# bababyVN/medical-image-segmentation-and-classification

Measured on AMD Instinct MI355X. Metric: images/sec (train step) Attention U-Net 256x256 bs=32/GPU, higher is better.
Workload: dtype bf16; 1 GPU; AttentionUNet 256x256 train step (fwd+BCE+bwd+clip+AdamW), bs=32/GPU, NHWC bf16 activations, fp32 master weights; global_batch=32, parallelism=dp1, hip_graph=False, wgrad_side_stream=True, plan_replay=C (mi355_plan_run)

## Files before the change

### include/mi355conv.h

```cpp
#ifndef MI355CONV_H_
#define MI355CONV_H_

#include <stdint.h>

#ifdef __cplusplus
extern "C" {
#endif

typedef struct ihipStream_t* mi355_stream_t;

enum { MI355_F32 = 0, MI355_BF16 = 1, MI355_F16 = 2 };
enum { MI355_OK = 0, MI355_ERR_ARG = -1, MI355_ERR_UNSUPPORTED = -2, MI355_ERR_RUNTIME = -3 };

int mi355_version(void);
const char* mi355_last_error(void);


int mi355_pack_input_nchw(const float* x, void* y, int N, int C, int H, int W, int Cpad, int dtype,
                          mi355_stream_t s);
int mi355_pack_input_im2col3(const float* x, void* y, int N, int C, int H, int W, int dtype, mi355_stream_t s);
int mi355_unpack_output_nchw(const void* x, float* y, int N, int C, int H, int W, int ld, int dtype,
                             mi355_stream_t s);
int mi355_pack_nchw(const float* x, void* y, int N, int C, int H, int W, int ld, int dtype, mi355_stream_t s);

int mi355_pack_conv_weight(const float* w, void* wf, void* wb, int Co, int Ci, int Cip, int KH, int KW,
                           int transposed, int dtype, mi355_stream_t s);

int mi355_pack_conv_weights_batched(const int64_t* table, int n, int fields ,
                                    int dtype, mi355_stream_t s);

int mi355_conv2d_igemm(const void* in, const void* wk, const float* bias, void* out,
                       int N, int Hi, int Wi, int Ci, int ldi,
                       int Ho, int Wo, int Co, int ldo,
                       int KH, int KW, int mul, int kmul, int off, int div, int up,
                       int accumulate, float* stats, int dtype, mi355_stream_t s);
int mi355_conv2d_igemm_variant(int Hi, int Wi, int Ci, int Ho, int Wo, int Co, int KH, int KW, int mul, int kmul, int off,
                               int div, int up, int dtype);
int mi355_conv2d_igemm_variant_n(int N, int Hi, int Wi, int Ci, int Ho, int Wo, int Co, int KH, int KW, int mul, int kmul,
                                 int off, int div, int up, int dtype);
int mi355_conv2d_igemm_dma_tile(int N, int Ho, int Wo, int Ci, int Co);
int mi355_conv2d_igemm_generic_tile(int N, int Ho, int Wo, int Co);
int mi355_conv2d_igemm_stat_rows(int N, int Hi, int Wi, int Ci, int Ho, int Wo, int Co, int KH, int KW,
                                 int mul, int kmul, int off, int div, int up, int dtype);
int mi355_conv2d_igemm_pool2_ok(int N, int Hi, int Wi, int Ci, int Ho, int Wo, int Co, int KH, int KW,
                                int mul, int kmul, int off, int div, int up, int dtype);
const char* mi355_conv2d_igemm_kernel_name(int N, int Hi, int Wi, int Ci, int Ho, int Wo, int Co, int KH, int KW,
                                           int mul, int kmul, int off, int div, int up, int dtype);

int mi355_conv2d_wgrad_splits(int N, int Ho, int Wo, int Ci, int Co, int KH, int KW);
int mi355_conv2d_wgrad_variant(int N, int Ho, int Wo, int KH, int KW, int stride, int pad, int dtype);
const char* mi355_conv2d_wgrad_kernel_name(int N, int Ho, int Wo, int Ci, int Co, int KH, int KW, int stride, int pad, int dtype);
int mi355_conv2d_wgrad(const void* x, const void* dy, float* ws, int splits,
                       int N, int Hi, int Wi, int Ci, int ldx,
                       int Ho, int Wo, int Co, int ldy,
                       int KH, int KW, int stride, int pad, int up, int dtype, mi355_stream_t s);
int mi355_conv2d_wgrad_multi_ok(int N, int Ho, int Wo, int dtype);
int mi355_conv2d_wgrad_multi(const void* x0, const void* dy0, const void* x1, const void* dy1, const void* x2, const void* dy2,
                             const void* x3, const void* dy3, const void* x4, const void* dy4, const void* x5, const void* dy5,
                             int napp, float* ws, int splits, int N, int Hi, int Wi, int Ci, int ldx, int Ho, int Wo, int Co,
                             int ldy, int up, int dtype, mi355_stream_t s);
int mi355_conv2d_wgrad_reduce(const float* ws, int splits, float* dw, int Co, int Ci, int Ci_real,
                              int KH, int KW, int transposed, float beta, mi355_stream_t s);


int mi355_rowreduce_blocks(long long M);
int mi355_bn_stats(const void* x, float* partial, long long M, int C, int ld, int dtype, mi355_stream_t s);
int mi355_bn_finalize(const float* partial, int nblocks, long long M, int C, const float* gamma,
                      const float* beta, float* running_mean, float* running_var, int64_t* nbt,
                      float momentum, float eps, float* scale, float* shift, float* mean, float* invstd,
                      mi355_stream_t s);
int mi355_fold_rows(const float* partial, int rows, int rowlen, float* out, int nsplit, mi355_stream_t s);
int mi355_bn_fold_bias(const float* bias, const float* scale, const float* shift, float* out, int C, mi355_stream_t s);
int mi355_bn_eval_coeffs(const float* gamma, const float* beta, const float* running_mean,
                         const float* running_var, float eps, int C, float* scale, float* shift,
                         mi355_stream_t s);
int mi355_bn_act(const void* x, int ldx, const float* scale, const float* shift,
                 const void* x2, int ldx2, const float* scale2, const float* shift2,
                 const void* res, int ldr, void* y, int ldy, long long M, int C, int act, int dtype,
                 mi355_stream_t s);
int mi355_bn_act_pool2(const void* x, int ldx, const float* scale, const float* shift, void* y, int ldy, void* p, int ldp,
                       int N, int H, int W, int C, int act, int dtype, mi355_stream_t s);
int mi355_bn_act_windows(const void* x, int ldx, const float* scale, const float* shift, const void* res, int ldr, void* y, int ldy,
                         int N, int H, int W, int C, int act, int dtype, mi355_stream_t s);
int mi355_bn_bwd_reduce_rows(long long M);
int mi355_bn_bwd_reduce(const void* dy, int lddy, const void* y, int ldy, const void* x, int ldx,
                        const float* mean, const float* invstd, const float* mscale, const float* mshift,
                        float* partial, long long M, int C, int act, int dtype, mi355_stream_t s);
int mi355_bn_bwd_finalize(const float* partial, int nblocks, int C, float* sums, float* dgamma, float* dbeta,
                          float acc, mi355_stream_t s);
int mi355_bn_bwd_finalize_at(const float* partial, int nblocks, int nq, int q0, int q1, int C, float* sums, float* dgamma,
                             float* dbeta, float acc, mi355_stream_t s);
int mi355_bn_bwd_apply(const void* dy, int lddy, const void* y, int ldy, const void* x, int ldx,
                       const float* gamma, const float* mean, const float* invstd, const float* mscale,
                       const float* mshift, const float* sums, void* dx, int lddx, void* dres, int lddres,
                       void* dpost, int lddpost, int post_acc, float* dbias_partial,
                       long long M, int C, int act, int dtype, mi355_stream_t s);
int mi355_bn_bwd_apply_post4(const void* dy, int lddy, const void* y, int ldy, const void* x, int ldx,
                             const float* gamma, const float* mean, const float* invstd, const float* mscale,
                             const float* mshift, const float* sums, void* dx, int lddx, void* dpost, int lddpost,
                             int post_acc, const void* ex0, const void* ex1, const void* ex2, const void* ex3, int ldex,
                             long long M, int C, int act, int dtype, mi355_stream_t s);
int mi355_bn_bwd_pool2_ok(int H, int W, int C, int dtype);
int mi355_bn_bwd_reduce_pool2_rows(long long M);
int mi355_bn_bwd_reduce_pool2(const void* dy, int lddy, const void* dp, int lddp, const void* x, int ldx, const float* mean,
                              const float* invstd, const float* mscale, const float* mshift, float* partial,
                              int N, int H, int W, int C, int dtype, mi355_stream_t s);
int mi355_bn_bwd_apply_pool2(const void* dy, int lddy, const void* dp, int lddp, const void* x, int ldx, const float* gamma,
                             const float* mean, const float* invstd, const float* mscale, const float* mshift,
                             const float* sums, void* dx, int lddx, int N, int H, int W, int C, int dtype, mi355_stream_t s);
int mi355_colsum_finalize(const float* partial, int nblocks, int stride, int C, float* out, float acc,
                          mi355_stream_t s);
int mi355_colsum(const void* x, int ld, float* partial, long long M, int C, int dtype, mi355_stream_t s);

int mi355_maxpool_fwd(const void* x, int ldx, void* y, int ldy, int N, int H, int W, int C,
                      int k, int stride, int pad, int dtype, mi355_stream_t s);
int mi355_maxpool_bwd(const void* x, int ldx, const void* dy, int lddy, void* dx, int lddx,
                      int N, int H, int W, int C, int k, int stride, int pad, int accumulate, int dtype,
                      mi355_stream_t s);
int mi355_upsample2_bwd(const void* dy, int lddy, void* dx, int lddx, int N, int H, int W, int C,
                        int accumulate, int dtype, mi355_stream_t s);
int mi355_add(const void* a, int lda, const void* b, int ldb, void* y, int ldy, long long M, int C, int dtype,
              mi355_stream_t s);
int mi355_relu_fwd(const void* x, int ldx, void* y, int ldy, long long M, int C, int dtype, mi355_stream_t s);
int mi355_relu_bwd(const void* dy, int lddy, const void* y, int ldy, void* dx, int lddx, long long M, int C,
                   int dtype, mi355_stream_t s);

int mi355_rowdot_fwd(const void* x, int ldx, const float* w, const float* b, float* z, float* partial,
                     long long M, int C, int HW, int K, int dtype, mi355_stream_t s);
int mi355_rowdot_bwd(const float* dz, const void* x, int ldx, const float* w, void* dx, int lddx,
                     float* partial, long long M, int C, int relu_mask, int HW, int K, int accumulate, int dtype,
                     mi355_stream_t s);
int mi355_gate_mul_fwd(const void* x, int ldx, const float* z, const float* scale, const float* shift,
                       void* y, int ldy, long long M, int C, int dtype, mi355_stream_t s);
int mi355_gate_mul_bwd(const void* dy, int lddy, const void* x, int ldx, const float* z, const float* scale,
// ... 125 lines not shown
```

### medical-image-segmentation-and-classification_amd/csrc/conv_wgrad.hip

```cpp
#include "common.hpp"
#include "dma.hpp"
#include "wgrad3x3_halo.hpp"
#include "wgrad3x3_halo8.hpp"
#include <stdlib.h>

struct WgradArgs {
  const void* x;
  const void* dy;
  float* ws;
  int N, Hi, Wi, Ci, ldx;
  int Ho, Wo, Co, ldy;
  int KH, KW, stride, pad, up;
  int M, Hlog, Wlog;
  int chunk;
};

typedef __attribute__((address_space(3))) s16x4 lds_s16x4;
template <typename T> struct TwoByte { typedef T type; };
template <> struct TwoByte<float> { typedef bf16_t type; };

template <typename T, int BCO, int BCI>
__global__ __launch_bounds__(256) void conv_wgrad_kernel(const WgradArgs a) {
  constexpr int BP = 32;
  constexpr int EPC = 16 / (int)sizeof(T);
  constexpr bool BF = sizeof(T) == 2;
  constexpr int PO = BF ? (BCO == 128 ? 320 : 192) : BCO * 4;
  constexpr int PX = BF ? (BCI == 128 ? 320 : 192) : BCI * 4;
  constexpr int O_BYTES = BP * PO, X_BYTES = BP * PX, STAGE = O_BYTES + X_BYTES;
  constexpr int CPRO = BCO / EPC, CPRX = BCI / EPC;
  constexpr int O_IT = BP * CPRO / 256, X_IT = BP * CPRX / 256;
  constexpr int WTO = BCO / 2, WTI = BCI / 2;
  constexpr int MI = WTO / 32, NI = WTI / 32;
  static_assert(O_IT >= 1 && X_IT >= 1, "tile too small for 256 threads");
  __shared__ __attribute__((aligned(16))) unsigned char lds[2 * STAGE];

  const int tid = threadIdx.x, lane = tid & 63, wave = tid >> 6;
  const int r32 = lane & 31, h = lane >> 5;
  const int wo_ = wave >> 1, wi_ = wave & 1;
  const int ciTiles = (a.Ci + BCI - 1) / BCI;
  int bid = xcd_tile((blockIdx.z * gridDim.y + blockIdx.y) * gridDim.x + blockIdx.x, gridDim.x * gridDim.y * gridDim.z);
  const int bx = bid % gridDim.x; bid /= gridDim.x;
  const int co0 = (bx / ciTiles) * BCO, ci0 = (bx % ciTiles) * BCI;
  const int tap = bid % gridDim.y, kh = tap / a.KW, kw = tap - kh * a.KW;
  const int split = bid / gridDim.y;
  const int p_begin = split * a.chunk;
  const int p_end = min(a.M, p_begin + a.chunk);
  const T* __restrict__ x = reinterpret_cast<const T*>(a.x);
  const T* __restrict__ dy = reinterpret_cast<const T*>(a.dy);

  int o_row[O_IT], o_c[O_IT];
#pragma unroll
  for (int i = 0; i < O_IT; ++i) {
    const int id = tid + i * 256;
    o_row[i] = id / CPRO;
    o_c[i] = id - o_row[i] * CPRO;
  }
  int x_row[X_IT], x_c[X_IT], x_n[X_IT], x_ho[X_IT], x_wo[X_IT];
  const int HoWo = a.Ho * a.Wo;
#pragma unroll
  for (int i = 0; i < X_IT; ++i) {
    const int id = tid + i * 256;
    x_row[i] = id / CPRX;
    x_c[i] = id - x_row[i] * CPRX;
    const int m = p_begin + x_row[i];
    x_n[i] = m / HoWo;
    const int rem = m - x_n[i] * HoWo;
    x_ho[i] = rem / a.Wo;
    x_wo[i] = rem - x_ho[i] * a.Wo;
  }

  uint4 ro[O_IT], rx[X_IT];
  auto load_tile = [&](int p0) {
#pragma unroll
    for (int i = 0; i < O_IT; ++i) {
      const int m = p0 + o_row[i];
      const int c = co0 + o_c[i] * EPC;
      if (m < p_end && c < a.Co)
        ro[i] = *reinterpret_cast<const uint4*>(dy + (size_t)m * a.ldy + c);
      else
        ro[i] = make_uint4(0, 0, 0, 0);
    }
#pragma unroll
    for (int i = 0; i < X_IT; ++i) {
      const int m = p0 + x_row[i];
      const int c = ci0 + x_c[i] * EPC;
      int th = x_ho[i] * a.stride + kh - a.pad, tw = x_wo[i] * a.stride + kw - a.pad;
// ... 152 lines not shown
  const long long max_by_pixels = M / 256 > 0 ? M / 256 : 1;
  if (s > max_by_pixels) s = max_by_pixels;
  const long long slab = (long long)Co * KH * KW * Ci * 4;
  while (s > 1 && s * slab > (512ll << 20)) --s;
  if (s < 1) s = 1;
  return (int)s;
}

template <typename T>
static int wgrad_launch(const WgradArgs& a, int splits, hipStream_t s) {
  int bco, bci;
  wgrad_tiles(a.Co, a.Ci, bco, bci);
  dim3 grid(ceil_div(a.Co, bco) * ceil_div(a.Ci, bci), a.KH * a.KW, splits);
  if (bco == 128 && bci == 128)
    hipLaunchKernelGGL((conv_wgrad_kernel<T, 128, 128>), grid, dim3(256), 0, s, a);
  else if (bco == 128)
    hipLaunchKernelGGL((conv_wgrad_kernel<T, 128, 64>), grid, dim3(256), 0, s, a);
  else if (bci == 128)
    hipLaunchKernelGGL((conv_wgrad_kernel<T, 64, 128>), grid, dim3(256), 0, s, a);
  else
    hipLaunchKernelGGL((conv_wgrad_kernel<T, 64, 64>), grid, dim3(256), 0, s, a);
  MI355_LAUNCH_CHECK();
  return MI355_OK;
}

template <typename T, bool W16>
static int launch_wgrad3x3(const Wgrad3Args& h, dim3 grid, hipStream_t s) {
  constexpr int lds_bytes = Wgrad3Lds<W16>::BYTES;
  static const hipError_t configured =
      hipFuncSetAttribute((const void*)wgrad3x3_halo_kernel<T, W16>, hipFuncAttributeMaxDynamicSharedMemorySize, lds_bytes);
  if (configured != hipSuccess)
    MI355_FAIL((int)configured, "wgrad3x3_halo: cannot reserve %d B of LDS: %s", lds_bytes, hipGetErrorString(configured));
  hipLaunchKernelGGL((wgrad3x3_halo_kernel<T, W16>), grid, dim3(256), lds_bytes, s, h);
  MI355_LAUNCH_CHECK();
  return MI355_OK;
}
template <typename T, bool W32>
static int launch_wgrad3x3_8(const Wgrad3Args& h, dim3 grid, hipStream_t s) {
  constexpr int lds_bytes = Wgrad8Lds::BYTES;
  static const hipError_t configured =
      hipFuncSetAttribute((const void*)wgrad3x3_halo8_kernel<T, W32>, hipFuncAttributeMaxDynamicSharedMemorySize, lds_bytes);
  if (configured != hipSuccess)
    MI355_FAIL((int)configured, "wgrad3x3_halo8: cannot reserve %d B of LDS: %s", lds_bytes, hipGetErrorString(configured));
  hipLaunchKernelGGL((wgrad3x3_halo8_kernel<T, W32>), grid, dim3(512), lds_bytes, s, h);
  MI355_LAUNCH_CHECK();
  return MI355_OK;
}
static int wgrad3_mode(int N, int Ho, int Wo, int KH, int KW, int stride, int pad, int dtype) {
  static const int use_halo = getenv("MI355_WGRAD_HALO") ? atoi(getenv("MI355_WGRAD_HALO")) : 1;
  if (!use_halo || !dtype_is_2byte(dtype) || stride != 1 || pad != 1) return 0;
  return halo_wgrad_mode(N, Ho, Wo, KH, KW);
}
static bool wgrad3_launchable(int hmode, int Hi, int Wi, int ldx, int Ho, int Wo, int ldy, int up, int esz) {
  const long long img_lim = (1ll << 31) / (hmode == 2 || hmode == 4 ? 2 : 1);
  return Ho == (up ? 2 * Hi : Hi) && Wo == (up ? 2 * Wi : Wi) && (long long)Hi * Wi * ldx * esz < img_lim && (long long)Ho * Wo * ldy * esz < img_lim;
}

static Wgrad3Args fill_wgrad3(const void* const* xs, const void* const* dys, int napp, float* ws, int hmode, int splits, int N, int Hi,
                              int Wi, int Ci, int ldx, int Ho, int Wo, int Co, int ldy, int up) {
  Wgrad3Args h;
  for (int i = 0; i < 6; ++i) { h.xs[i] = xs[i < napp ? i : 0]; h.dys[i] = dys[i < napp ? i : 0]; }
  h.ws = ws;
  h.N = N; h.Hi = Hi; h.Wi = Wi; h.Ci = Ci; h.ldx = ldx;
  h.H = Ho; h.W = Wo; h.Co = Co; h.ldy = ldy; h.up = up ? 1 : 0;
  h.RB = Ho % 32 == 0 ? 32 : (Ho % 16 == 0 ? 16 : 8);
  h.items_per_app = halo_wgrad_items(hmode, N, Ho, Wo, h.RB);
  h.items = napp * h.items_per_app;
  h.items_per_block = ceil_div(h.items, splits);
  return h;
}

static const char* wgrad3_name(int hmode) { return hmode >= 3 ? "wgrad3x3_halo8_kernel" : "wgrad3x3_halo_kernel"; }
static int launch_wgrad3(const Wgrad3Args& h, int splits, int hmode, int dtype, hipStream_t s) {
  const dim3 grid(ceil_div(h.Co, 64) * ceil_div(h.Ci, 64), splits);
  const bool f16 = dtype == MI355_F16;
  switch (hmode) {
    case 2: return f16 ? launch_wgrad3x3<f16_t, true>(h, grid, s) : launch_wgrad3x3<bf16_t, true>(h, grid, s);
    case 3: return f16 ? launch_wgrad3x3_8<f16_t, false>(h, grid, s) : launch_wgrad3x3_8<bf16_t, false>(h, grid, s);
    case 4: return f16 ? launch_wgrad3x3_8<f16_t, true>(h, grid, s) : launch_wgrad3x3_8<bf16_t, true>(h, grid, s);
    default: return f16 ? launch_wgrad3x3<f16_t, false>(h, grid, s) : launch_wgrad3x3<bf16_t, false>(h, grid, s);
  }
}

extern "C" int mi355_conv2d_wgrad_variant(int N, int Ho, int Wo, int KH, int KW, int stride, int pad, int dtype) {
  return wgrad3_mode(N, Ho, Wo, KH, KW, stride, pad, dtype);
}
extern "C" int mi355_conv2d_wgrad_multi_ok(int N, int Ho, int Wo, int dtype) { return wgrad3_mode(N, Ho, Wo, 3, 3, 1, 1, dtype) ? 1 : 0; }
extern "C" const char* mi355_conv2d_wgrad_kernel_name(int N, int Ho, int Wo, int Ci, int Co, int KH, int KW, int stride, int pad, int dtype) {
  static thread_local char name[48];
  if (const int hmode = wgrad3_mode(N, Ho, Wo, KH, KW, stride, pad, dtype)) return wgrad3_name(hmode);
  int bco, bci;
  wgrad_tiles(Co, Ci, bco, bci);
  snprintf(name, sizeof(name), "conv_wgrad_kernel<%s,%d,%d>", dtype_is_2byte(dtype) ? "bf16" : "f32", bco, bci);
  return name;
}

extern "C" int mi355_conv2d_wgrad(const void* x, const void* dy, float* ws, int splits, int N, int Hi, int Wi, int Ci,
                                  int ldx, int Ho, int Wo, int Co, int ldy, int KH, int KW, int stride, int pad, int up,
                                  int dtype, mi355_stream_t s) {
  MI355_CHECK_ARG(x && dy && ws, "conv2d_wgrad: null pointer");
  MI355_CHECK_ARG(splits >= 1 && splits <= 65535, "conv2d_wgrad: splits=%d out of range", splits);
  const int esz = dtype_is_2byte(dtype) ? 2 : 4;
  const int epc = 16 / esz;
  MI355_CHECK_ARG(Ci % epc == 0 && Co % epc == 0, "conv2d_wgrad: Ci=%d / Co=%d must be multiples of %d", Ci, Co, epc);
  MI355_CHECK_ARG(((uintptr_t)x % 16) == 0 && ((uintptr_t)dy % 16) == 0 && (ldx * esz) % 16 == 0 && (ldy * esz) % 16 == 0,
                  "conv2d_wgrad: pointers / channel strides must be 16-byte aligned");
  MI355_CHECK_ARG((long long)N * Ho * Wo < (1ll << 31) && (long long)N * Hi * Wi < (1ll << 31),
                  "conv2d_wgrad: pixel count overflows int32");
  const int hmode = wgrad3_mode(N, Ho, Wo, KH, KW, stride, pad, dtype);
  if (hmode && wgrad3_launchable(hmode, Hi, Wi, ldx, Ho, Wo, ldy, up, esz))
    return launch_wgrad3(fill_wgrad3(&x, &dy, 1, ws, hmode, splits, N, Hi, Wi, Ci, ldx, Ho, Wo, Co, ldy, up), splits, hmode, dtype, (hipStream_t)s);
  WgradArgs a;
  a.x = x; a.dy = dy; a.ws = ws;
  a.N = N; a.Hi = Hi; a.Wi = Wi; a.Ci = Ci; a.ldx = ldx;
  a.Ho = Ho; a.Wo = Wo; a.Co = Co; a.ldy = ldy;
  a.KH = KH; a.KW = KW; a.stride = stride; a.pad = pad; a.up = up ? 1 : 0;
  a.M = N * Ho * Wo; a.Hlog = up ? 2 * Hi : Hi; a.Wlog = up ? 2 * Wi : Wi;
  a.chunk = ceil_div(ceil_div(a.M, splits), 32) * 32;
  return dispatch_dtype(dtype, "conv2d_wgrad", [&](auto tag) { return wgrad_launch<decltype(tag)>(a, splits, (hipStream_t)s); });
}

extern "C" int mi355_conv2d_wgrad_multi(const void* x0, const void* dy0, const void* x1, const void* dy1, const void* x2,
                                        const void* dy2, const void* x3, const void* dy3, const void* x4, const void* dy4,
                                        const void* x5, const void* dy5, int napp, float* ws, int splits, int N, int Hi, int Wi,
                                        int Ci, int ldx, int Ho, int Wo, int Co, int ldy, int up, int dtype, mi355_stream_t s) {
  const void* xs[6] = {x0, x1, x2, x3, x4, x5};
  const void* dys[6] = {dy0, dy1, dy2, dy3, dy4, dy5};
  MI355_CHECK_ARG(napp >= 1 && napp <= 6 && ws && splits >= 1, "conv2d_wgrad_multi: 1..6 operand pairs, a workspace, splits >= 1");
  for (int i = 0; i < napp; ++i)
    MI355_CHECK_ARG(xs[i] && dys[i] && ((uintptr_t)xs[i] % 16) == 0 && ((uintptr_t)dys[i] % 16) == 0,
                    "conv2d_wgrad_multi: pair %d: null or misaligned pointer", i);
  const int hmode = wgrad3_mode(N, Ho, Wo, 3, 3, 1, 1, dtype);
  MI355_CHECK_ARG(hmode, "conv2d_wgrad_multi: shape / dtype not served by the nine-tap kernel "
                  "(mi355_conv2d_wgrad_multi_ok == 0): run mi355_conv2d_wgrad per pair");
  MI355_CHECK_ARG(Ci % 8 == 0 && Co % 8 == 0 && (ldx * 2) % 16 == 0 && (ldy * 2) % 16 == 0 && ldx >= Ci && ldy >= Co,
                  "conv2d_wgrad_multi: channel counts / strides must be multiples of 8 elements");
  MI355_CHECK_ARG((up ? (Ho == 2 * Hi && Wo == 2 * Wi) : (Ho == Hi && Wo == Wi)), "conv2d_wgrad_multi: 3x3 / stride 1 / pad 1 geometry only");
  MI355_CHECK_ARG((long long)Hi * Wi * ldx * 4 < (1ll << 31) && (long long)Ho * Wo * ldy * 4 < (1ll << 31),
                  "conv2d_wgrad_multi: an image of 1 GiB or more is beyond the 32-bit offsets of the nine-tap kernel's buffer descriptors");
  const Wgrad3Args h = fill_wgrad3(xs, dys, napp, ws, hmode, splits, N, Hi, Wi, Ci, ldx, Ho, Wo, Co, ldy, up);
  MI355_CHECK_ARG(splits <= h.items, "conv2d_wgrad_multi: more splits (%d) than work items (%d)", splits, h.items);
  return launch_wgrad3(h, splits, hmode, dtype, (hipStream_t)s);
}


#define WR_CI 32
template <int TAPS>
__global__ __launch_bounds__(1024) void wgrad_reduce_kernel(const float* __restrict__ ws, int splits, float* __restrict__ dw, int Co,
                                                            int Ci, int Ci_real, int taps_rt, int transposed, float beta, int KL) {
  extern __shared__ float tile[];
  const int taps = TAPS > 0 ? TAPS : taps_rt;
  const int ciTiles = (Ci + WR_CI - 1) / WR_CI;
  const int co = blockIdx.x / ciTiles, ci0 = (blockIdx.x % ciTiles) * WR_CI;
  const size_t total = (size_t)Co * taps * Ci;
  const int cl = threadIdx.x % WR_CI, kl = threadIdx.x / WR_CI;
  const int ci = ci0 + cl;
  const int tstride = taps * (WR_CI + 1);
  if constexpr (TAPS > 0) {
    float s0[TAPS], s1[TAPS];
#pragma unroll
    for (int tap = 0; tap < TAPS; ++tap) { s0[tap] = 0.f; s1[tap] = 0.f; }
    if (ci < Ci) {
      const float* p = ws + (size_t)co * TAPS * Ci + ci;
      int k = kl;
      for (; k + KL < splits; k += 2 * KL) {
        float a[TAPS], b[TAPS];
#pragma unroll
        for (int tap = 0; tap < TAPS; ++tap) {
          a[tap] = p[(size_t)k * total + (size_t)tap * Ci];
          b[tap] = p[(size_t)(k + KL) * total + (size_t)tap * Ci];
        }
#pragma unroll
        for (int tap = 0; tap < TAPS; ++tap) { s0[tap] += a[tap]; s1[tap] += b[tap]; }
      }
      if (k < splits) {
#pragma unroll
        for (int tap = 0; tap < TAPS; ++tap) s0[tap] += p[(size_t)k * total + (size_t)tap * Ci];
      }
    }
#pragma unroll
    for (int tap = 0; tap < TAPS; ++tap) tile[kl * tstride + tap * (WR_CI + 1) + cl] = s0[tap] + s1[tap];
  } else {
    for (int tap = 0; tap < taps; ++tap) {
      float s0 = 0.f, s1 = 0.f;
      if (ci < Ci) {
        const float* p = ws + ((size_t)co * taps + tap) * Ci + ci;
        int k = kl;
        for (; k + KL < splits; k += 2 * KL) {
          s0 += p[(size_t)k * total];
          s1 += p[(size_t)(k + KL) * total];
        }
        if (k < splits) s0 += p[(size_t)k * total];
      }
      tile[kl * tstride + tap * (WR_CI + 1) + cl] = s0 + s1;
    }
  }
  __syncthreads();
  const int n = taps * WR_CI;
  for (int t = threadIdx.x; t < n; t += WR_CI * KL) {
    const int c2 = t / taps, tap = t - c2 * taps;
    const int cc = ci0 + c2;
    if (cc >= Ci_real) continue;
    float s = 0.f;
    for (int k = 0; k < KL; ++k) s += tile[k * tstride + tap * (WR_CI + 1) + c2];
    const size_t o = transposed ? ((size_t)cc * Co + co) * taps + tap : ((size_t)co * Ci_real + cc) * taps + tap;
    dw[o] = (beta != 0.f ? beta * dw[o] : 0.f) + s;
  }
}

extern "C" int mi355_conv2d_wgrad_reduce(const float* ws, int splits, float* dw, int Co, int Ci, int Ci_real, int KH,
                                         int KW, int transposed, float beta, mi355_stream_t s) {
  MI355_CHECK_ARG(ws && dw && splits >= 1, "conv2d_wgrad_reduce: bad arguments");
  const int taps = KH * KW;
  const int ciTiles = (Ci + WR_CI - 1) / WR_CI;
  int KL = 15000 / (taps * (WR_CI + 1));
  if (KL > 32) KL = 32;
  if (KL > splits) KL = splits;
  if (KL < 1) KL = 1;
  const dim3 grid(Co * ciTiles), block(WR_CI * KL);
  const size_t lds = KL * taps * (WR_CI + 1) * sizeof(float);
  if (taps == 9)
    hipLaunchKernelGGL(wgrad_reduce_kernel<9>, grid, block, lds, (hipStream_t)s, ws, splits, dw, Co, Ci, Ci_real, taps, transposed, beta, KL);
  else
    hipLaunchKernelGGL(wgrad_reduce_kernel<0>, grid, block, lds, (hipStream_t)s, ws, splits, dw, Co, Ci, Ci_real, taps, transposed, beta, KL);
// ... 4 lines not shown
```

### medical-image-segmentation-and-classification_amd/mi355/graph.py

```python
from __future__ import annotations

import ctypes
import os
import struct
from typing import List, Optional

import torch
import torch.nn as nn

from .lib import lib, DTYPE_CODE

BN_EPS_DEFAULT = 1e-5
CPAD = 32
FUSE_POOL = os.environ.get("MI355_FUSE_POOL", "1") != "0"
FUSE_POOL_BWD = os.environ.get("MI355_FUSE_POOL_BWD", "1") != "0"
FUSE_GATE_BWD = os.environ.get("MI355_FUSE_GATE_BWD", "1") != "0"
FUSE_HEAD = os.environ.get("MI355_FUSE_HEAD", "1") != "0"
STEM_IM2COL = os.environ.get("MI355_STEM_IM2COL", "1") != "0"
SIDE_COLSUM = os.environ.get("MI355_SIDE_COLSUM", "1") != "0"
BN_ACT_WINDOWS = os.environ.get("MI355_BN_ACT_WINDOWS", "1") != "0"
STATIC_PACKS = os.environ.get("MI355_STATIC_PACKS", "1") != "0"
BN_ACT_WINDOWS_RES = os.environ.get("MI355_BN_ACT_WINDOWS_RES", "1") != "0"
FUSE_RESIDUAL = os.environ.get("MI355_FUSE_RESIDUAL", "1") != "0"
DEFER_POST = os.environ.get("MI355_DEFER_POST", "1") != "0"
# ... 467 lines not shown
        N, C, H, W = t.N, t.C, t.H, t.W
        out = self.f32(N * C * H * W)
        self.fwd.append(Launch("mi355_unpack_output_nchw", t, out, N, C, H, W, t.ld, self.code))
        self.output = ("z", out, (N, C, H, W))
        if self.want_grad and t.needs_grad:
            self.dout = self.f32(N * C * H * W)

            def rule():
                if self.acc_flag(t):
                    raise NotImplementedError("tensor_output of an activation with other consumers")
                g = self.grad_of(t)
                self.bwd.append(Launch("mi355_pack_nchw", self.dout, g, N, C, H, W, g.ld, self.code))
            self.rule(rule)
        return out

    def packs(self, conv, cip, transposed=False, scale=None):
        key = (id(conv), cip, id(scale))
        if key not in self._packs:
            w = conv.weight
            if transposed:
                ci, co = w.shape[0], w.shape[1]
            else:
                co, ci = w.shape[0], w.shape[1]
            k = w.shape[2]
            if hasattr(conv, "pack_shape"):
                co, ci, k = conv.pack_shape
            wf = self._alloc(co * k * k * cip)
            wb = self._alloc(co * k * k * cip) if self.want_grad else None
            assert k * k <= 288, "batched weight pack: at most 288 taps"
            self._pack_table.append((w, wf, wb, co, ci, cip, k * k, 1 if transposed else 0, scale))
            self.see(w, conv.bias)
            self._packs[key] = (wf, wb)
        return self._packs[key]

    def _conv_geom(self, x, conv, up):
        k, s, p = conv.kernel_size[0], conv.stride[0], conv.padding[0]
        if conv.kernel_size[0] != conv.kernel_size[1] or conv.dilation[0] != 1 or conv.groups != 1:
            raise NotImplementedError("square, undilated, ungrouped convolutions only")
        hl, wl = (2 * x.H, 2 * x.W) if up else (x.H, x.W)
        return k, s, p, (hl + 2 * p - k) // s + 1, (wl + 2 * p - k) // s + 1

    def conv_raw(self, x, conv, up=False, out=None, stats=False, relu=False, fold=None):
        stem = self._stem_as_pointwise(x, conv, up)
        if stem is not None:
            return self.conv_raw(stem[0], stem[1], out=out, stats=stats, relu=relu, fold=fold)
        if x is getattr(self, "_xin", None):
            self._xin_users += 1
        k, s, p, Ho, Wo = self._conv_geom(x, conv, up)
        Co = conv.out_channels
        assert x.C >= conv.in_channels and (x.C == conv.in_channels or conv.in_channels < CPAD), (x.C, conv.in_channels)
        wf, wb = self.packs(conv, x.C, scale=fold[0] if fold else None)
        bias = fold[1] if fold else conv.bias
        y = out if out is not None else self.new_tensor(x.N, Ho, Wo, Co)
        assert (y.N, y.H, y.W, y.C) == (x.N, Ho, Wo, Co)
        flops = 2 * x.N * Ho * Wo * Co * k * k * conv.in_channels
        nbytes = (x.N * x.H * x.W * x.C + x.N * Ho * Wo * Co + Co * k * k * x.C) * self.esz
        stat_part = None
        self._last_stat_rows = 0
        geom = (x.N, x.H, x.W, x.C, Ho, Wo, Co, k, k, s, 1, -p, 1, 1 if up else 0)
        if stats and self.training:
            rows = lib.mi355_conv2d_igemm_stat_rows(*geom, self.code)
            if rows > 0:
                stat_part = self.ws_f32(rows * 2 * Co)
                self._last_stat_rows = rows
        self.fwd.append(self.igemm(x, wf, bias, y, geom, 2 if relu else 0, stat_part, flops=flops, nbytes=nbytes))
        y.needs_grad = x.needs_grad or self.param_grad(conv.weight)
        self._conv_uses[id(conv)] = self._conv_uses.get(id(conv), 0) + 1

        def bwd(dy, bias_done=False):
            uses = self._conv_uses[id(conv)]
            if (self.param_grad(conv.weight) and 1 < uses <= 6 and self.multi_wgrad and k == 3 and s == 1 and p == 1 and self.esz == 2
                    and lib.mi355_conv2d_wgrad_multi_ok(x.N, Ho, Wo, self.code)):
                pend = self._pending_wgrad.setdefault(id(conv), [])
                pend.append((x, dy))
                assert (x.N, x.H, x.W, x.C, x.ld, dy.ld) == tuple(getattr(pend[0][0], f) for f in ("N", "H", "W", "C", "ld")) + (pend[0][1].ld,)
                if len(pend) == uses:
                    self._emit_multi_wgrad(conv, pend, Ho, Wo, Co, k, up, flops, nbytes)
                    del self._pending_wgrad[id(conv)]
            elif self.param_grad(conv.weight):
                splits = lib.mi355_conv2d_wgrad_splits(x.N, Ho, Wo, x.C, Co, k, k)
                ws = self.ws_bytes(splits * Co * k * k * x.C * 4)
                self.bwd.append(Launch("mi355_conv2d_wgrad", x, dy, ws, splits, x.N, x.H, x.W, x.C, x.ld, Ho, Wo, Co, dy.ld,
                                       k, k, s, p, 1 if up else 0, self.code, flops=flops, nbytes=nbytes, side=True,
                                       tag=self.wgrad_tag(Co, x.C, k, s, Ho, Wo, x.N, p), cus=self.wgrad_cus(x.N, Ho, Wo, x.C, Co, k, s, p, splits)))
                ref, beta = self.pgrad(conv.weight)
                self.bwd.append(Launch("mi355_conv2d_wgrad_reduce", ws, splits, ref, Co, x.C, conv.in_channels, k, k, 0, beta, side=True))
            if conv.bias is not None and self.param_grad(conv.bias) and not bias_done:
                self.bias_grad_from(dy, conv.bias)
            if x.needs_grad:
                acc = self.acc_flag(x)
                xg = self.grad_of(x)
                hg, wg = (2 * x.H, 2 * x.W) if up else (x.H, x.W)
                dgeom = (x.N, Ho, Wo, Co, hg, wg, x.C, k, k, 1, -1, p, s, 0)
                if not up:
                    self.bwd.append(self.igemm(dy, wb, None, xg, dgeom, acc, flops=flops, nbytes=nbytes))
                elif lib.mi355_conv2d_igemm_pool2_ok(*dgeom, self.code):
                    self.bwd.append(self.igemm(dy, wb, None, xg, dgeom, 4 | (1 if acc else 0), flops=flops, nbytes=nbytes))
                else:
                    tmp = self.new_tensor(x.N, hg, wg, x.C)
                    self.bwd.append(self.igemm(dy, wb, None, tmp, dgeom, 0, flops=flops, nbytes=nbytes))
                    self.bwd.append(Launch("mi355_upsample2_bwd", tmp, tmp.ld, xg, xg.ld, x.N, x.H, x.W, x.C, acc, self.code))
        return y, bwd

    def _emit_multi_wgrad(self, conv, pend, Ho, Wo, Co, k, up, flops, nbytes):
        x0 = pend[0][0]
        n = len(pend)
        splits = lib.mi355_conv2d_wgrad_splits(x0.N * n, Ho, Wo, x0.C, Co, k, k)
        ws = self.ws_bytes(splits * Co * k * k * x0.C * 4)
        ops = []
        for i in range(6):
            ops += list(pend[i]) if i < n else [None, None]
        self.bwd.append(Launch("mi355_conv2d_wgrad_multi", *ops, n, ws, splits, x0.N, x0.H, x0.W, x0.C, x0.ld, Ho, Wo, Co,
                               pend[0][1].ld, 1 if up else 0, self.code, flops=flops * n, nbytes=nbytes * n, side=True,
                               tag=self.wgrad_tag(Co, x0.C, k, 1, Ho, Wo, x0.N, 1), cus=self.wgrad_cus(x0.N, Ho, Wo, x0.C, Co, k, 1, 1, splits)))
        ref, beta = self.pgrad(conv.weight)
        self.bwd.append(Launch("mi355_conv2d_wgrad_reduce", ws, splits, ref, Co, x0.C, conv.in_channels, k, k, 0, beta, side=True))

    def igemm(self, x, w, bias, out, geom, flags=0, stats=None, **kw):
        return Launch("mi355_conv2d_igemm", x, w, bias, out, *geom[:4], x.ld, *geom[4:7], out.ld, *geom[7:], flags, stats, self.code,
                      tag=self.igemm_tag(geom), **kw)

    def igemm_tag(self, geom):
        return lib.mi355_conv2d_igemm_kernel_name(*geom, self.code).decode()

    def wgrad_tag(self, co, ci, k=1, s=1, Ho=0, Wo=0, N=0, p=None):
        return lib.mi355_conv2d_wgrad_kernel_name(N, Ho, Wo, ci, co, k, k, s, (k // 2) if p is None else p, self.code).decode()

    def wgrad_cus(self, N, Ho, Wo, ci, co, k, s, p, splits):
        if self.esz != 2 or lib.mi355_conv2d_wgrad_variant(N, Ho, Wo, k, k, s, p, self.code) < 3:
            return 1.0
        return min(1.0, -(-co // 64) * -(-ci // 64) * splits / 256.0)

    def bias_grad_from(self, dy, bias):
        nb = lib.mi355_rowreduce_blocks(dy.M)
        part = self.ws_f32(nb * dy.C)
        self.bwd.append(Launch("mi355_colsum", dy, dy.ld, part, dy.M, dy.C, self.code))
        ref, beta = self.pgrad(bias)
        self.bwd.append(Launch("mi355_colsum_finalize", part, nb, 1, dy.C, ref, beta))

    def _bn_coeffs(self, y, bn, fused_rows=0):
        C = bn.num_features
        st = {k: self.f32(C) for k in ("scale", "shift", "mean", "invstd")}
        self.see(bn.weight, bn.bias)
        if self.training:
            if fused_rows > 0:
                nb = fused_rows
                part = self.ws_f32(nb * 2 * C)
                if nb > 2048:
                    folded = self.f32(64 * 2 * C)
                    self.fwd.append(Launch("mi355_fold_rows", part, nb, 2 * C, folded, 64))
                    part, nb = folded, 64
            else:
                nb = lib.mi355_rowreduce_blocks(y.M)
                part = self.ws_f32(nb * 2 * C)
                self.fwd.append(Launch("mi355_bn_stats", y, part, y.M, C, y.ld, self.code))
            mom = bn.momentum if bn.momentum is not None else 0.1
            track = bn.track_running_stats
            self.fwd.append(Launch("mi355_bn_finalize", part, nb, y.M, C, bn.weight, bn.bias,
                                   bn.running_mean if track else None, bn.running_var if track else None,
                                   bn.num_batches_tracked if track else None, float(mom), float(bn.eps),
                                   st["scale"], st["shift"], st["mean"], st["invstd"]))
        else:
            self.fwd.append(Launch("mi355_bn_eval_coeffs", bn.weight, bn.bias, bn.running_mean, bn.running_var, float(bn.eps),
                                   C, st["scale"], st["shift"]))
        return st

    def _bn_bwd(self, da, a, y, bn, st, act, dres_to=None, bias=None, post_to=None, pool_dp=None, head=None):
        C = bn.num_features
        nb = lib.mi355_rowreduce_blocks(y.M)
        part = self.ws_f32(nb * 2 * C)
        if head is not None:
            dz, hconv = head
            assert act and dres_to is None and post_to is None and pool_dp is None
            part = self.f32(nb * 5 * C) if SIDE_COLSUM else self.ws_f32(nb * 5 * C)
            co = (st["scale"], st["shift"], st["mean"], st["invstd"], None, None, None, None)
            self.bwd.append(Launch("mi355_gate_bn_bwd_reduce", dz, y, y.ld, None, 0, *co, hconv.weight, part, y.M, C, self.code,
                                   nbytes=y.M * C * self.esz + 4 * y.M))
            head_folds = []
            if self.param_grad(hconv.weight):
                wref, wbeta = self.pgrad(hconv.weight)
                head_folds.append(Launch("mi355_colsum_finalize", self._ws_off(part, 3 * C * 4), nb, 5, C, wref, wbeta, side=SIDE_COLSUM))
                if hconv.bias is not None:
                    bref2, bbeta = self.pgrad(hconv.bias)
                    head_folds.append(Launch("mi355_colsum_finalize", self._ws_off(part, 4 * C * 4), nb, 5 * C, 1, bref2, bbeta, side=SIDE_COLSUM))
            sums = self.f32(2 * C)
            need_pg = self.param_grad(bn.weight)
            if need_pg:
                gref, gbeta = self.pgrad(bn.weight)
                bref, _ = self.pgrad(bn.bias)
            self.bwd.append(Launch("mi355_bn_bwd_finalize_at", part, min(nb, lib.mi355_gate_bn_bwd_reduce_rows(y.M)), 5, 0, 1, C, sums,
                                   gref if need_pg else None, bref if need_pg else None, gbeta if need_pg else 0.0))
            if bias is not None and self.param_grad(bias) and id(bias) not in self._grad_first:
                self.pgrad(bias)
                self.zero_grad_params.append(bias)
            dy = self.grad_of(y)
            self.bwd.append(Launch("mi355_gate_bn_bwd_apply", dz, y, y.ld, None, 0, *co, hconv.weight, bn.weight, None, sums, None,
                                   dy, dy.ld, None, 0, y.M, C, self.code, nbytes=2 * y.M * C * self.esz + 4 * y.M))
            self.bwd += head_folds
            return dy
        if pool_dp is not None:
            assert act and dres_to is None and post_to is None
            dal = da.ld if da is not None else 0
            self.bwd.append(Launch("mi355_bn_bwd_reduce_pool2", da, dal, pool_dp, pool_dp.ld, y, y.ld, st["mean"], st["invstd"],
                                   st["scale"], st["shift"], part, y.N, y.H, y.W, C, self.code,
                                   nbytes=int((1.25 + (da is not None)) * y.M * C * self.esz)))
            sums = self.f32(2 * C)
            need_pg = self.param_grad(bn.weight)
            if need_pg:
# ... 632 lines not shown
```

Baseline: 2127 images/s.

## Add phase-decomposed wgrad kernel for 3x3 convs on 2x-upsampled inputs

Adds a new weight-gradient kernel for 3x3 convolutions whose input is a nearest 2x upsample. It splits the output into four sub-pixel phases and reads the low-resolution input directly, so each phase collapses the nine taps into a 2x2 group of accumulators. This removes redundant MFMA work and the reads of the upsampled tensor. The kernel uses a 512-thread block with a large dynamic LDS ring and exchanges half-tiles before writing per-tap partials. It adds code complexity and changes the write pattern to read-modify-write across phases.

```diff
diff --git a/include/mi355conv.h b/include/mi355conv.h
--- a/include/mi355conv.h
+++ b/include/mi355conv.h
@@ -50,6 +50,7 @@
 int mi355_conv2d_wgrad_splits(int N, int Ho, int Wo, int Ci, int Co, int KH, int KW);
 int mi355_conv2d_wgrad_variant(int N, int Ho, int Wo, int KH, int KW, int stride, int pad, int dtype);
 const char* mi355_conv2d_wgrad_kernel_name(int N, int Ho, int Wo, int Ci, int Co, int KH, int KW, int stride, int pad, int dtype);
+const char* mi355_conv2d_wgrad_up_kernel_name(int N, int Hi, int Wi, int Ci, int Co, int up, int dtype);
 int mi355_conv2d_wgrad(const void* x, const void* dy, float* ws, int splits,
                        int N, int Hi, int Wi, int Ci, int ldx,
                        int Ho, int Wo, int Co, int ldy,
diff --git a/medical-image-segmentation-and-classification_amd/csrc/conv_wgrad.hip b/medical-image-segmentation-and-classification_amd/csrc/conv_wgrad.hip
--- a/medical-image-segmentation-and-classification_amd/csrc/conv_wgrad.hip
+++ b/medical-image-segmentation-and-classification_amd/csrc/conv_wgrad.hip
@@ -2,6 +2,7 @@
 #include "dma.hpp"
 #include "wgrad3x3_halo.hpp"
 #include "wgrad3x3_halo8.hpp"
+#include "wgrad_up_phase8.hpp"
 #include <stdlib.h>
 
 struct WgradArgs {
@@ -320,6 +321,44 @@
   }
 }
 
+static int wgrad_up_mode(int N, int Hi, int Wi, int up, int dtype) {
+  static const int use_phases = getenv("MI355_WGRAD_UP_PHASES") ? atoi(getenv("MI355_WGRAD_UP_PHASES")) : 1;
+  if (!use_phases || !up || Hi <= 0 || Wi <= 0 || Hi % 8 != 0 || wgrad3_mode(N, 2 * Hi, 2 * Wi, 3, 3, 1, 1, dtype) < 3) return -1;
+  if (Wi % 64 == 0) return 0;
+  if (Wi == 32 && N % 2 == 0) return 1;
+  if (Wi == 16 && N % 4 == 0) return 2;
+  return -1;
+}
+static bool wgrad_up_launchable(int umode, int Hi, int Wi, int ldx, int Ho, int Wo, int ldy, int esz) {
+  const long long img_lim = (1ll << 31) >> umode;
+  return Ho == 2 * Hi && Wo == 2 * Wi && (long long)Hi * Wi * ldx * esz < img_lim && (long long)Ho * Wo * ldy * esz < img_lim;
+}
+static const char* wgrad_up_name() { return "wgrad_up_phase8_kernel"; }
+template <typename T, int MODE>
+static int launch_wgrad_up_t(const Wgrad3Args& h, dim3 grid, hipStream_t s) {
+  constexpr int lds_bytes = WgradUpLds<MODE>::BYTES;
+  static const hipError_t configured =
+      hipFuncSetAttribute((const void*)wgrad_up_phase8_kernel<T, MODE>, hipFuncAttributeMaxDynamicSharedMemorySize, lds_bytes);
+  if (configured != hipSuccess)
+    MI355_FAIL((int)configured, "wgrad_up_phase8: cannot reserve %d B of LDS: %s", lds_bytes, hipGetErrorString(configured));
+  hipLaunchKernelGGL((wgrad_up_phase8_kernel<T, MODE>), grid, dim3(512), lds_bytes, s, h);
+  MI355_LAUNCH_CHECK();
+  return MI355_OK;
+}
+static int launch_wgrad_up(Wgrad3Args h, int napp, int splits, int umode, int dtype, hipStream_t s) {
+  h.RB = h.Hi % 32 == 0 ? 32 : (h.Hi % 16 == 0 ? 16 : 8);
+  h.items_per_app = (umode == 0 ? h.N * (h.Wi / 64) : h.N >> umode) * (h.Hi / h.RB);
+  h.items = napp * h.items_per_app;
+  h.items_per_block = ceil_div(h.items, splits);
+  const dim3 grid(ceil_div(h.Co, 64) * ceil_div(h.Ci, 64), splits);
+  const bool f16 = dtype == MI355_F16;
+  switch (umode) {
+    case 0: return f16 ? launch_wgrad_up_t<f16_t, 0>(h, grid, s) : launch_wgrad_up_t<bf16_t, 0>(h, grid, s);
+    case 1: return f16 ? launch_wgrad_up_t<f16_t, 1>(h, grid, s) : launch_wgrad_up_t<bf16_t, 1>(h, grid, s);
+    default: return f16 ? launch_wgrad_up_t<f16_t, 2>(h, grid, s) : launch_wgrad_up_t<bf16_t, 2>(h, grid, s);
+  }
+}
+
 extern "C" int mi355_conv2d_wgrad_variant(int N, int Ho, int Wo, int KH, int KW, int stride, int pad, int dtype) {
   return wgrad3_mode(N, Ho, Wo, KH, KW, stride, pad, dtype);
 }
@@ -331,6 +370,11 @@
   wgrad_tiles(Co, Ci, bco, bci);
   snprintf(name, sizeof(name), "conv_wgrad_kernel<%s,%d,%d>", dtype_is_2byte(dtype) ? "bf16" : "f32", bco, bci);
   return name;
+}
+
+extern "C" const char* mi355_conv2d_wgrad_up_kernel_name(int N, int Hi, int Wi, int Ci, int Co, int up, int dtype) {
+  if (wgrad_up_mode(N, Hi, Wi, up, dtype) >= 0) return wgrad_up_name();
+  return mi355_conv2d_wgrad_kernel_name(N, up ? 2 * Hi : Hi, up ? 2 * Wi : Wi, Ci, Co, 3, 3, 1, 1, dtype);
 }
 
 extern "C" int mi355_conv2d_wgrad(const void* x, const void* dy, float* ws, int splits, int N, int Hi, int Wi, int Ci,
@@ -346,6 +390,9 @@
   MI355_CHECK_ARG((long long)N * Ho * Wo < (1ll << 31) && (long long)N * Hi * Wi < (1ll << 31),
                   "conv2d_wgrad: pixel count overflows int32");
   const int hmode = wgrad3_mode(N, Ho, Wo, KH, KW, stride, pad, dtype);
+  const int umode = wgrad_up_mode(N, Hi, Wi, up, dtype);
+  if (umode >= 0 && wgrad_up_launchable(umode, Hi, Wi, ldx, Ho, Wo, ldy, esz))
+    return launch_wgrad_up(fill_wgrad3(&x, &dy, 1, ws, hmode, splits, N, Hi, Wi, Ci, ldx, Ho, Wo, Co, ldy, up), 1, splits, umode, dtype, (hipStream_t)s);
   if (hmode && wgrad3_launchable(hmode, Hi, Wi, ldx, Ho, Wo, ldy, up, esz))
     return launch_wgrad3(fill_wgrad3(&x, &dy, 1, ws, hmode, splits, N, Hi, Wi, Ci, ldx, Ho, Wo, Co, ldy, up), splits, hmode, dtype, (hipStream_t)s);
   WgradArgs a;
@@ -378,6 +425,8 @@
                   "conv2d_wgrad_multi: an image of 1 GiB or more is beyond the 32-bit offsets of the nine-tap kernel's buffer descriptors");
   const Wgrad3Args h = fill_wgrad3(xs, dys, napp, ws, hmode, splits, N, Hi, Wi, Ci, ldx, Ho, Wo, Co, ldy, up);
   MI355_CHECK_ARG(splits <= h.items, "conv2d_wgrad_multi: more splits (%d) than work items (%d)", splits, h.items);
+  const int umode = wgrad_up_mode(N, Hi, Wi, up, dtype);
+  if (umode >= 0 && wgrad_up_launchable(umode, Hi, Wi, ldx, Ho, Wo, ldy, 2)) return launch_wgrad_up(h, napp, splits, umode, dtype, (hipStream_t)s);
   return launch_wgrad3(h, splits, hmode, dtype, (hipStream_t)s);
 }
 
diff --git a/medical-image-segmentation-and-classification_amd/csrc/wgrad_up_phase8.hpp b/medical-image-segmentation-and-classification_amd/csrc/wgrad_up_phase8.hpp
--- /dev/null
+++ b/medical-image-segmentation-and-classification_amd/csrc/wgrad_up_phase8.hpp
@@ -0,0 +1,272 @@
+#pragma once
+#include <type_traits>
+#include "common.hpp"
+#include "dma.hpp"
+#include "wgrad3x3_halo.hpp"
+
+template <int MODE> struct WgradUpLds {
+  static constexpr int NR = 6;
+  static constexpr int XPX = MODE == 2 ? 96 : 80, DPX = 64;
+  static constexpr int BYTES = NR * (XPX + DPX) * 128;
+};
+
+template <typename T, int MODE>
+__global__ __launch_bounds__(512, 2) void wgrad_up_phase8_kernel(const Wgrad3Args a) {
+  static_assert(sizeof(T) == 2, "bf16 / fp16 only");
+  using L = WgradUpLds<MODE>;
+  constexpr int XPX = L::XPX, XROW = XPX * 128, DROW = L::DPX * 128;
+  constexpr int XSEG = MODE == 0 ? 72 : (MODE == 1 ? 40 : 24);
+  constexpr int XPIECES = MODE == 0 ? 9 : (MODE == 1 ? 10 : 12);
+  constexpr int NIMG = MODE == 0 ? 1 : (MODE == 1 ? 2 : 4);
+  constexpr int DSEG = 64 / NIMG;
+  constexpr int NR = L::NR, PF = 5;
+  constexpr int X_BYTES = NR * XROW, D_BYTES = NR * DROW;
+  static_assert(L::BYTES == X_BYTES + D_BYTES, "launcher and kernel disagree on the LDS size");
+
+  extern __shared__ __attribute__((aligned(16))) unsigned char lds[];
+  const unsigned lds_x = lds_addr(lds), lds_d = lds_addr(lds + X_BYTES);
+
+  const int tid = threadIdx.x, lane = tid & 63, wave = __builtin_amdgcn_readfirstlane(tid >> 6);
+  const int half = wave >> 2, w4 = wave & 3;
+  const int l16 = lane & 15, c4 = lane >> 4;
+  const int qo = w4 >> 1, qi = w4 & 1;
+  const int ciTiles = (a.Ci + 63) / 64;
+  const int bid = xcd_tile(blockIdx.y * gridDim.x + blockIdx.x, gridDim.x * gridDim.y);
+  const int bx = bid % gridDim.x, by = bid / gridDim.x;
+  int tco = bx / ciTiles, tci = bx % ciTiles;
+  {
+    const int coT = gridDim.x / ciTiles, Q = (int)(gridDim.x * gridDim.y) >> 3;
+    if (Q >= 4 && (int)gridDim.x % Q == 0 && ((gridDim.x * gridDim.y) & 7) == 0) {
+      int BW = 0, best = 1 << 30;
+      for (int w = 1; w <= Q; w <<= 1) {
+        const int h = Q / w;
+        if (w * h == Q && ciTiles % w == 0 && coT % h == 0 && w + h < best) { best = w + h; BW = w; }
+      }
+      if (BW) {
+        const int BH = Q / BW, blk = bx / Q, j = bx % Q, bpr = ciTiles / BW;
+        tco = (blk / bpr) * BH + j / BW;
+        tci = (blk % bpr) * BW + j % BW;
+      }
+    }
+  }
+  const int co0 = tco * 64, ci0 = tci * 64;
+  auto swz = [](int px) { return (((px >> 1) & 1) | (((px >> 3) & 1) << 1)) << 1; };
+
+  const int lpx = lane >> 3, slot = lane & 7;
+  const int TXN = MODE == 0 ? a.Wi / 64 : 1, BANDS = a.Hi / a.RB;
+  const bool three = 8 + wave < XPIECES;
+
+  const int tq = l16 >> 2, tp = l16 & 3;
+  const int pl = 8 * c4 + tq;
+  const int plx = MODE == 0 ? 32 * half + pl : (MODE == 1 ? 40 * half + pl : 48 * half + 24 * (c4 >> 1) + 8 * (c4 & 1) + tq);
+  const int dhalf = half * 32 * 128;
+  auto rd = [&](int img_off, int px, int col) {
+    const int chunk = (col >> 3) ^ swz(px);
+    return __builtin_amdgcn_ds_read_tr16_b64_v4i16((lds_s16x4_t*)(lds + img_off + px * 128 + chunk * 16 + (col & 7) * 2));
+  };
+  auto frag = [&](int img_off, int px, int col) {
+    const s16x4 v0 = rd(img_off, px, col), v1 = rd(img_off, px + 4, col);
+    return __builtin_bit_cast(bf16x8, __builtin_shufflevector(v0, v1, 0, 1, 2, 3, 4, 5, 6, 7));
+  };
+  const int colA = qo * 32 + 4 * tp, colB = qi * 32 + 4 * tp;
+
+  const int item0 = by * a.items_per_block;
+  const int item1 = min(a.items, item0 + a.items_per_block);
+  float* __restrict__ ws = a.ws + (size_t)by * a.Co * 9 * a.Ci;
+  float4* const xch = reinterpret_cast<float4*>(lds) + w4 * 64 + lane;
+  static_assert(4 * 4 * 256 * 16 <= X_BYTES + D_BYTES, "the half-tile exchange fits in the dead rings");
+
+#pragma unroll 1
+  for (int phase = 0; phase < 4; ++phase) {
+    const int py = phase >> 1, px = phase & 1;
+    f32x4 acc[2][2][2][2];
+#pragma unroll
+    for (int g = 0; g < 4; ++g)
+#pragma unroll
+      for (int i = 0; i < 2; ++i)
+#pragma unroll
+        for (int j = 0; j < 2; ++j) acc[g >> 1][g & 1][i][j] = f32x4{0.f, 0.f, 0.f, 0.f};
+
+    for (int item = item0; item < item1; ++item) {
+      const int app = item / a.items_per_app;
+      const T* __restrict__ x = reinterpret_cast<const T*>(a.xs[app]);
+      const T* __restrict__ dy = reinterpret_cast<const T*>(a.dys[app]);
+      int t = item - app * a.items_per_app;
+      const int band = t % BANDS; t /= BANDS;
+      const int tx = t % TXN;
+      const int n = t / TXN;
+      const int ia = band * a.RB, ib = ia + a.RB, x0 = tx * 64;
+      const int nbase = NIMG * n;
+      const int px_d = 8 * wave + lpx;
+      const int c_d = co0 + 8 * (slot ^ swz(px_d));
+      const bool lane_ok_d = c_d < a.Co;
+      const int dpix = MODE == 0 ? 2 * (x0 + px_d) : (px_d / DSEG) * a.H * a.W + 2 * (px_d % DSEG);
+      int xpix[2], c_x[2], xpiece[2];
+      bool lane_ok_x[2];
+#pragma unroll
+      for (int k = 0; k < 2; ++k) {
+        xpiece[k] = k == 0 ? wave : 8 + wave;
+        const int q = 8 * xpiece[k] + lpx;
+        const int hq = MODE == 0 ? 0 : q / XSEG;
+        const int xx = MODE == 0 ? x0 - 4 + q + px : q % XSEG - 4 + px;
+        c_x[k] = ci0 + 8 * (slot ^ swz(q));
+        lane_ok_x[k] = xpiece[k] < XPIECES && (unsigned)xx < (unsigned)a.Wi && c_x[k] < a.Ci;
+        xpix[k] = hq * a.Hi * a.Wi + xx;
+      }
+
+      const bufdesc_t desc_d = make_buf(dy + (size_t)nbase * a.H * a.W * a.ldy);
+      const bufdesc_t desc_x = make_buf(x + (size_t)nbase * a.Hi * a.Wi * a.ldx);
+      const unsigned voff_d = lane_ok_d ? (unsigned)((dpix * a.ldy + c_d) * (int)sizeof(T)) : DMA_PAD;
+      unsigned voff_x[2];
+#pragma unroll
+      for (int k = 0; k < 2; ++k) voff_x[k] = lane_ok_x[k] ? (unsigned)((xpix[k] * a.ldx + c_x[k]) * (int)sizeof(T)) : DMA_PAD;
+      const unsigned d_stride = (unsigned)(2 * a.W * a.ldy) * (unsigned)sizeof(T), x_stride = (unsigned)(a.Wi * a.ldx) * (unsigned)sizeof(T);
+      const unsigned d_base = (unsigned)((py * a.W + px) * a.ldy) * (unsigned)sizeof(T);
+      auto with_rows = [](bufdesc_t d, bool ok) { d[2] = ok ? (int)DMA_PAD : 0; return d; };
+      int k_next = 0;
+      unsigned d_soff_next = d_base + (unsigned)ia * d_stride, x_soff_next = (unsigned)(ia - 1 + py) * x_stride;
+      auto issue_next_piece = [&](int piece, int sl) {
+        if (piece == 0) {
+          dma16_buf(with_rows(desc_d, ia + k_next < ib), voff_d, d_soff_next, lds_d + sl * DROW + wave * 1024);
+        } else if (piece == 1 || three) {
+          const int k = piece - 1;
+          dma16_buf(with_rows(desc_x, (unsigned)(ia - 1 + py + k_next) < (unsigned)a.Hi), voff_x[k], x_soff_next, lds_x + sl * XROW + xpiece[k] * 1024);
+        }
+        if (piece == 2) {
+          d_soff_next += d_stride;
+          x_soff_next += x_stride;
+          ++k_next;
+        }
+      };
+      auto load_x = [&](int sl, int c, bf16x8 (&bf)[2]) {
+#pragma unroll
+        for (int bi = 0; bi < 2; ++bi) bf[bi] = frag(sl * XROW, plx + 3 + c, colB + 16 * bi);
+      };
+      auto load_dy = [&](int sl, bf16x8 (&af)[2]) {
+#pragma unroll
+        for (int ao = 0; ao < 2; ++ao) af[ao] = frag(X_BYTES + sl * DROW + dhalf, pl, colA + 16 * ao);
+      };
+      bf16x8 da[2], db[2], dn[2];
+      auto mfma4 = [&](int g, int c, const bf16x8 (&dg)[2], const bf16x8 (&xk)[2]) {
+#pragma unroll
+        for (int ao = 0; ao < 2; ++ao)
+#pragma unroll
+          for (int bi = 0; bi < 2; ++bi) mfma_16x16x32_acc<T>(dg[ao], xk[bi], acc[g][c][ao][bi]);
+      };
+
+#pragma unroll
+      for (int k = 0; k < PF; ++k)
+#pragma unroll
+        for (int piece = 0; piece < 3; ++piece) issue_next_piece(piece, k);
+      if (three) wait_vmcnt<3 * (PF - 2)>(); else wait_vmcnt<2 * (PF - 2)>();
+      __builtin_amdgcn_s_barrier();
+
+      bf16x8 xa[2], xb[2];
+      load_x(0, 0, xa);
+      load_dy(0, db);
+#pragma unroll
+      for (int ao = 0; ao < 2; ++ao) da[ao] = __builtin_bit_cast(bf16x8, make_uint4(0, 0, 0, 0));
+      auto row_step = [&](auto slot_tag) {
+        constexpr int S = decltype(slot_tag)::value;
+        constexpr int SN = (S + PF) % NR;
+        load_x(S, 1, xb);
+        __builtin_amdgcn_sched_barrier(0);
+        mfma4(0, 0, da, xa);
+        issue_next_piece(0, SN);
+        mfma4(1, 0, db, xa);
+        issue_next_piece(1, SN);
+        __builtin_amdgcn_sched_barrier(0);
+        asm volatile("s_waitcnt lgkmcnt(0)" ::: "memory");
+        if (three) wait_vmcnt<3 * (PF - 2) + 2>(); else wait_vmcnt<2 * (PF - 2) + 2>();
+        __builtin_amdgcn_s_barrier();
+        load_x((S + 1) % NR, 0, xa);
+        load_dy((S + 1) % NR, dn);
+        __builtin_amdgcn_sched_barrier(0);
+        mfma4(0, 1, da, xb);
+        issue_next_piece(2, SN);
+        mfma4(1, 1, db, xb);
+#pragma unroll
+        for (int ao = 0; ao < 2; ++ao) {
+          da[ao] = db[ao];
+          db[ao] = dn[ao];
+        }
+      };
+      using S0 = std::integral_constant<int, 0>;
+      using S1 = std::integral_constant<int, 1>;
+      using S2 = std::integral_constant<int, 2>;
+      using S3 = std::integral_constant<int, 3>;
+      using S4 = std::integral_constant<int, 4>;
+      using S5 = std::integral_constant<int, 5>;
+      static_assert(NR == 6, "six step bodies per trip");
+      int s = 0;
+      for (; s + 6 <= a.RB + 1; s += 6) {
+        row_step(S0{});
+        row_step(S1{});
+        row_step(S2{});
+        row_step(S3{});
+        row_step(S4{});
+        row_step(S5{});
+      }
+      row_step(S0{});
+      row_step(S1{});
+      row_step(S2{});
+      if (s + 5 <= a.RB + 1) {
+        row_step(S3{});
+        row_step(S4{});
+      }
+      asm volatile("s_waitcnt lgkmcnt(0)" ::: "memory");
+      wait_vmcnt<0>();
+      __builtin_amdgcn_s_barrier();
+    }
+
+    mfma_results_ready();
+    if (half == 1) {
+#pragma unroll
+      for (int g = 0; g < 4; ++g)
+#pragma unroll
+        for (int ao = 0; ao < 2; ++ao)
+#pragma unroll
+          for (int bi = 0; bi < 2; ++bi) {
+            const f32x4 v = acc[g >> 1][g & 1][ao][bi];
+            xch[((g * 2 + ao) * 2 + bi) * 256] = make_float4(v[0], v[1], v[2], v[3]);
+          }
+    }
+    __syncthreads();
+    if (half == 0) {
+#pragma unroll
+      for (int g = 0; g < 4; ++g) {
+        const int gy = g >> 1, gx = g & 1;
+        const int kh0 = gy == 0 ? 1 + py : 0, kh1 = gy == 0 ? 2 : py;
+        const int kw0 = gx == 0 ? 0 : px + 1, kw1 = gx == 0 ? px : 2;
+        f32x4 v[2][2];
+#pragma unroll
+        for (int ao = 0; ao < 2; ++ao)
+#pragma unroll
+          for (int bi = 0; bi < 2; ++bi) {
+            const float4 o = xch[((g * 2 + ao) * 2 + bi) * 256];
+            v[ao][bi] = acc[gy][gx][ao][bi] + f32x4{o.x, o.y, o.z, o.w};
+          }
+#pragma unroll 1
+        for (int kh = kh0; kh <= kh1; ++kh)
+#pragma unroll 1
+          for (int kw = kw0; kw <= kw1; ++kw) {
+            const int tap = kh * 3 + kw;
+#pragma unroll
+            for (int ao = 0; ao < 2; ++ao)
+#pragma unroll
+              for (int bi = 0; bi < 2; ++bi)
+#pragma unroll
+                for (int r = 0; r < 4; ++r) {
+                  const int co = co0 + qo * 32 + ao * 16 + 4 * c4 + r;
+                  const int ci = ci0 + qi * 32 + bi * 16 + l16;
+                  if (co < a.Co && ci < a.Ci) {
+                    float* p = ws + ((size_t)co * 9 + tap) * a.Ci + ci;
+                    *p = phase == 0 ? v[ao][bi][r] : *p + v[ao][bi][r];
+                  }
+                }
+          }
+      }
+    }
+    __syncthreads();
+  }
+}
diff --git a/medical-image-segmentation-and-classification_amd/mi355/graph.py b/medical-image-segmentation-and-classification_amd/mi355/graph.py
--- a/medical-image-segmentation-and-classification_amd/mi355/graph.py
+++ b/medical-image-segmentation-and-classification_amd/mi355/graph.py
@@ -573,7 +573,7 @@
                 ws = self.ws_bytes(splits * Co * k * k * x.C * 4)
                 self.bwd.append(Launch("mi355_conv2d_wgrad", x, dy, ws, splits, x.N, x.H, x.W, x.C, x.ld, Ho, Wo, Co, dy.ld,
                                        k, k, s, p, 1 if up else 0, self.code, flops=flops, nbytes=nbytes, side=True,
-                                       tag=self.wgrad_tag(Co, x.C, k, s, Ho, Wo, x.N, p), cus=self.wgrad_cus(x.N, Ho, Wo, x.C, Co, k, s, p, splits)))
+                                       tag=self.wgrad_tag(Co, x.C, k, s, Ho, Wo, x.N, p, up), cus=self.wgrad_cus(x.N, Ho, Wo, x.C, Co, k, s, p, splits)))
                 ref, beta = self.pgrad(conv.weight)
                 self.bwd.append(Launch("mi355_conv2d_wgrad_reduce", ws, splits, ref, Co, x.C, conv.in_channels, k, k, 0, beta, side=True))
             if conv.bias is not None and self.param_grad(conv.bias) and not bias_done:
@@ -603,7 +603,7 @@
             ops += list(pend[i]) if i < n else [None, None]
         self.bwd.append(Launch("mi355_conv2d_wgrad_multi", *ops, n, ws, splits, x0.N, x0.H, x0.W, x0.C, x0.ld, Ho, Wo, Co,
                                pend[0][1].ld, 1 if up else 0, self.code, flops=flops * n, nbytes=nbytes * n, side=True,
-                               tag=self.wgrad_tag(Co, x0.C, k, 1, Ho, Wo, x0.N, 1), cus=self.wgrad_cus(x0.N, Ho, Wo, x0.C, Co, k, 1, 1, splits)))
+                               tag=self.wgrad_tag(Co, x0.C, k, 1, Ho, Wo, x0.N, 1, up), cus=self.wgrad_cus(x0.N, Ho, Wo, x0.C, Co, k, 1, 1, splits)))
         ref, beta = self.pgrad(conv.weight)
         self.bwd.append(Launch("mi355_conv2d_wgrad_reduce", ws, splits, ref, Co, x0.C, conv.in_channels, k, k, 0, beta, side=True))
 
@@ -614,7 +614,9 @@
     def igemm_tag(self, geom):
         return lib.mi355_conv2d_igemm_kernel_name(*geom, self.code).decode()
 
-    def wgrad_tag(self, co, ci, k=1, s=1, Ho=0, Wo=0, N=0, p=None):
+    def wgrad_tag(self, co, ci, k=1, s=1, Ho=0, Wo=0, N=0, p=None, up=False):
+        if up and k == 3 and s == 1 and p == 1:
+            return lib.mi355_conv2d_wgrad_up_kernel_name(N, Ho // 2, Wo // 2, ci, co, 1, self.code).decode()
         return lib.mi355_conv2d_wgrad_kernel_name(N, Ho, Wo, ci, co, k, k, s, (k // 2) if p is None else p, self.code).decode()
 
     def wgrad_cus(self, N, Ho, Wo, ci, co, k, s, p, splits):
```

Result: no change. 2137 images/s, median of 6 (+0.5%).
